# Maofei/loam_velodyne-1

Measured on AMD Instinct MI355X. Metric: scans/sec (odometry+mapping L-M solve) VLP-16 sweep, 1/2/4/8 MI355X, higher is better.
Workload: dtype fp32 (fp64 JtJ accumulation); 1 GPU; config4: independent VLP-16 problems (SR prev+cur, odometry L-M, mapping L-M); problems_per_gpu=1024, global_batch=1024, split=strong, parallelism=shard1

## Files before the change

### loam_velodyne-1_amd/csrc/dev_hooks.h

```cpp
#ifndef LOAM_DEV_HOOKS_H
#define LOAM_DEV_HOOKS_H

#include <stdint.h>

#ifdef __cplusplus
extern "C" {
#endif

typedef struct loam_dev_vg loam_dev_vg;

#define LOAM_DEV_VG_STACK 0
#define LOAM_DEV_VG_CUBES 1
#define LOAM_DEV_VG_SURROUND 2

typedef struct {
  const float* pts;
  int32_t total;
  int32_t nseg;
  const int32_t* begin;
  const int32_t* end;
  const float* leaf;
  const int32_t* nold;
  int32_t route;
  int32_t P;
// ... 15 lines not shown
#define LOAM_DEV_NN5_MAX_QUERIES 4096
#define LOAM_DEV_NN5_BATCH 0
#define LOAM_DEV_NN5_STREAM 1
#define LOAM_DEV_NN5_OVERFLOW 1
#define LOAM_DEV_NN5_PLAIN 2

typedef struct {
  const float* map;
  int32_t n_map;
  const float* queries;
  int32_t n_queries;
  const int32_t* seeds;
  const int32_t* distinct;
  int32_t form;
} loam_dev_nn5_job;

int loam_dev_nn5_create(int device, loam_dev_nn5** out);

int loam_dev_nn5_run(loam_dev_nn5* h, const loam_dev_nn5_job* job, int32_t* flat_idx, uint32_t* flat_dist,
                     int32_t* plain_idx, uint32_t* plain_dist, int32_t* flags, int32_t* counts);

int loam_dev_nn5_destroy(loam_dev_nn5* h);

#ifdef __cplusplus
}
#endif
#endif
```

### loam_velodyne-1_amd/csrc/engine.hpp

```cpp
#ifndef LOAM_ENGINE_HPP
#define LOAM_ENGINE_HPP

#include <hip/hip_runtime.h>
#include <stdint.h>

#include <cstring>
#include <string>

#include "../../include/loam/loam.h"
#include "imu.hpp"
#include "prof.hpp"

namespace loam {

enum : int {
  ERR_CAP_RING = 1,
  ERR_CAP_ROWS = 2,
  ERR_EMPTY = 4,
  ERR_CAP_MAP = 8,
  ERR_CAP_STACK = 16,
  ERR_VG_BITS = 32,
};

constexpr int kSrThreads = 512;
// ... 7 lines not shown
  int od_fused_max = 128;
  int mp_small_max = 4;
  int mp_fused_max = 1 << 20;
  int od_assoc_wg = 0;
  int fit_wg = 0;
  int graph = 0;
  int vg_merge = 1;
  int vg_merge_min = 12288;
  int vg_split = 1;
  int sr_ahead = 64;
  int step_pipe = 64;
  int pipe_mp_sets = 2;
  int od_graph = 1;
  int pipe_sr_sets = 3;
  int batch_streams = 1;
  int sr_ahead_at = -1;
  int od_sel_min = 64;
  int od_win_mono = 3;
  int od_win_mono_min = 2;
  int stream_defer = 1;
  int od_persist = 1;
  int mp_persist = 1;
  int od_moments_min = 64;
  bool get(const char* key, long long* v) {
    return set(key, 0, v);
  }
  bool set(const char* key, long long v, long long* read = nullptr) {
    struct K { const char* n; int* f; long long lo, hi; };
    const K ks[] = {{"od_small_max", &od_small_max, 0, 1 << 20}, {"stream_defer", &stream_defer, 0, 1}, {"pipe_sr_sets", &pipe_sr_sets, 2, 3}, {"od_graph", &od_graph, 0, 1},
                    {"od_fused_max", &od_fused_max, 0, 1 << 20},
                    {"mp_small_max", &mp_small_max, 0, 1 << 20}, {"mp_fused_max", &mp_fused_max, 0, 1 << 20},
                    {"od_assoc_wg", &od_assoc_wg, 0, 1024}, {"fit_wg", &fit_wg, 0, 256}, {"graph", &graph, 0, 1},
                    {"vg_merge", &vg_merge, 0, 1}, {"vg_merge_min", &vg_merge_min, 0, 1 << 20}, {"vg_split", &vg_split, 0, 3},
                    {"sr_ahead", &sr_ahead, 0, 1 << 20}, {"sr_ahead_at", &sr_ahead_at, -1, 2},
                    {"step_pipe", &step_pipe, 0, 1 << 20}, {"batch_streams", &batch_streams, 0, 1},
                    {"pipe_mp_sets", &pipe_mp_sets, 1, 2}, {"od_sel_min", &od_sel_min, 1, 1 << 20},
                    {"od_win_mono", &od_win_mono, 0, 3}, {"od_win_mono_min", &od_win_mono_min, 1, 1 << 20},
                    {"od_moments_min", &od_moments_min, 1, 1 << 30}, {"od_persist", &od_persist, 0, 1},
                    {"mp_persist", &mp_persist, 0, 1}};
    for (const K& k : ks)
      if (std::strcmp(key, k.n) == 0) {
        if (read) {
          *read = *k.f;
          return true;
        }
        if (v < k.lo || v > k.hi) return false;
        *k.f = (int)v;
        return true;
      }
    return false;
  }
};

struct SrBuffers {
  int S = 0, cap = 0, R = 0;
  float4* raw = nullptr;
  int* raw_n = nullptr;
  float* tmp_ori = nullptr;
  uint8_t* tmp_sid = nullptr;
  int* tilecnt = nullptr;
  int* tileF = nullptr;
  int* ring_sync = nullptr;
// ... 141 lines not shown
```

### loam_velodyne-1_amd/csrc/od.hip

```cpp
#include "dev_common.hpp"
#include "od.hpp"
#include "pose_math.hpp"

using namespace loamdev;


#ifndef LOAM_ASSOC_SKIP
#define LOAM_ASSOC_SKIP 0
#endif
#ifndef LOAM_ASSOC_PHASE
#define LOAM_ASSOC_PHASE 0
#endif
#if (LOAM_ASSOC_SKIP != 0 || LOAM_ASSOC_PHASE != 0) && !defined(LOAM_EXPERIMENT_BUILD)
#error "LOAM_ASSOC_SKIP / LOAM_ASSOC_PHASE are diagnostic (wrong results / partial counters): tools/build_variant.sh only"
#endif

namespace loam {
#ifdef LOAM_PHASES
__device__ PhaseAcc g_ph_od = {~0ull, 0ull, 0ull, {{0}}};
#endif


namespace {

// ... 286 lines not shown
  hipLaunchKernelGGL(k_hash_scan, dim3(1, P, 2), dim3(1024), 0, st, hp);
  hipLaunchKernelGGL(k_hash_scatter, dim3(kHashGrid, P, 2), dim3(256), 0, st, hp);
}

namespace {


LOAM_D float box_d2(const float4& lo, const float4& hi, const float4& s) {
  const float gx = fmaxf(fmaxf(lo.x - s.x, s.x - hi.x), 0.0f);
  const float gy = fmaxf(fmaxf(lo.y - s.y, s.y - hi.y), 0.0f);
  const float gz = fmaxf(fmaxf(lo.z - s.z, s.z - hi.z), 0.0f);
  return sqdist(gx, gy, gz, 0.0f, 0.0f, 0.0f);
}

LOAM_D bool window_member(int j, int r, int c, int scan, int fwd_end, bool corner, bool same) {
  if (j > c) return j < fwd_end && r <= scan + 2 && (corner ? r > scan : (same ? r <= scan : r > scan));
  return j < c && r >= scan - 2 && (corner ? r < scan : (same ? r >= scan : r < scan));
}

struct WinBound {
  float same = 25.0f, other = 25.0f;
};

LOAM_D uint64_t wave_hash_nn(const int* start, const float4* hp, int T, const float4* cloud, const float4* ch,
                             int n, float h, float inv_h, float4 q, float bound, int* cells, int& wpts, int& wbox,
                             int kind = -1, int fwd_end = 0, bool mono = false, WinBound* wb = nullptr) {
  const int lane = lane_id();
  const int cx = cell_of(q.x, inv_h), cy = cell_of(q.y, inv_h), cz = cell_of(q.z, inv_h);
  int bucket = -1, b0 = 0, cnt = 0;
  if (lane < 27 && T > 0) {
    const int dx = lane % 3 - 1, dy = (lane / 3) % 3 - 1, dz = lane / 9 - 1;
    const float4 lo = make_float4((float)(cx + dx) * h, (float)(cy + dy) * h, (float)(cz + dz) * h, 0.0f);
    const float4 hi = make_float4((float)(cx + dx + 1) * h, (float)(cy + dy + 1) * h, (float)(cz + dz + 1) * h, 0.0f);
    const float bd = box_d2(lo, hi, q);
    if (h != 1.0f || (bd < 1.0f && bd <= bound)) {
      bucket = (int)(cell_hash(cx + dx, cy + dy, cz + dz) & (uint32_t)(T - 1));
      const int2 rg = load_pair(start + bucket);
      b0 = rg.x;
      cnt = rg.y - b0;
      LOAM_CHECK(b0 >= 0 && cnt >= 0 && b0 + cnt <= n, b0, cnt);
    }
  }
  const int incl = wave_incl_scan_x(cnt);
  const int total = __builtin_amdgcn_readlane(incl, 63);
  if (LOAM_ASSOC_PHASE == 0 || LOAM_ASSOC_PHASE == 1) wpts += total;
  if (lane < 32) { cells[lane] = lane < 27 ? incl - cnt : 0x7fffffff; cells[32 + lane] = b0; }
// ... 21 lines not shown
  if (best != ~0ull && __uint_as_float((uint32_t)(best >> 32)) < h * h) {
    if (kind >= 0 && mono && D(__uint_as_float((uint32_t)(best >> 32))) < 25) {
      const int c = (int)((uint32_t)best >> 8), scan = (int)((uint32_t)best & 255u);
      float ms = 3.4e38f, mo = 3.4e38f;
      for (int t = lane; t < total; t += 64) {
        const float4 a = t == lane ? a0 : cand(t);
        const uint32_t tag = (uint32_t)__float_as_int(a.w);
        const int j = (int)(tag & 0xffffffu), r = (int)(tag >> 24);
        const float d = sqdist(a.x, a.y, a.z, q.x, q.y, q.z);
        if (kind == 0) {
          if (window_member(j, r, c, scan, fwd_end, true, false)) mo = fminf(mo, d);
        } else if (window_member(j, r, c, scan, fwd_end, false, true)) {
          ms = fminf(ms, d);
        } else if (window_member(j, r, c, scan, fwd_end, false, false)) {
          mo = fminf(mo, d);
        }
      }
      wb->same = fminf(wb->same, wave_min_f_x(ms));
      wb->other = fminf(wb->other, wave_min_f_x(mo));
    }
    return best;
  }
  if (LOAM_ASSOC_SKIP & 2) return best;
  best = ~0ull;
  const int nch = (n + kChunk - 1) / kChunk;
  for (int k0 = 0; k0 < nch; k0 += 64) {
    const int k = k0 + lane;
    float bd = 0.0f;
    if (k < nch) bd = box_d2(ch[2 * k], ch[2 * k + 1], q);
    const bool need = k < nch && bd < 25.0f && bd <= bound;
    uint64_t nb = __ballot(need);
    wbox += min(64, nch - k0);
    while (nb) {
      const int c = k0 + __ffsll((unsigned long long)nb) - 1;
      nb &= nb - 1;
      if (LOAM_ASSOC_PHASE == 0 || LOAM_ASSOC_PHASE == 2) wpts += min(kChunk, n - c * kChunk);
      const int t = c * kChunk + lane;
      if (lane < kChunk && t < n) {
        const float4 a = cloud[t];
        const float d = sqdist(a.x, a.y, a.z, q.x, q.y, q.z);
        const uint64_t key = ((uint64_t)fkey(d) << 32) | ((uint32_t)t << 8) | (uint32_t)(int)a.w;
        best = key < best ? key : best;
      }
    }
  }
  return wave_min_u64_x(best);
}

#ifndef LOAM_WIN_INFLIGHT
#define LOAM_WIN_INFLIGHT 1
#endif
constexpr int kWinInFlight = LOAM_WIN_INFLIGHT;
template <typename F>
LOAM_D void wave_window(const float4* L, const float4* ch, int c, int end, int dir, int scan, float4 sel, float bs,
                        float bo, int& wpts, int& wbox, F f) {
  const int lane = lane_id();
  auto stop_ring = [&](int r) { return dir > 0 ? r > scan + 2 : r < scan - 2; };
  auto scan_pts = [&](int j0, int cnt, float4 a) {
    if (LOAM_ASSOC_PHASE == 0 || LOAM_ASSOC_PHASE == 3) wpts += cnt;
    const int j = j0 + dir * lane;
    const bool inr = lane < cnt;
    const int r = (int)a.w;
    const uint64_t mb = __ballot(inr && stop_ring(r));
    const int limit = mb ? __ffsll((unsigned long long)mb) - 1 : 64;
    if (inr && lane < limit) {
      const float d = sqdist(a.x, a.y, a.z, sel.x, sel.y, sel.z);
      if (d < 25) f(j, r, d);
    }
    return mb != 0;
// ... 279 lines not shown
  ist[kIsNanSkips] = 0;
  ist[kIsGathered] = 0;
  ist[kIsBoxes] = 0;
  b.done[p] = 0;
  if (p == 0 && b.P == 1) ++b.ls_epoch[0];
}

__global__ __launch_bounds__(kOdThreads) void k_od_sel(OdBuffers b, FeatView f) {
  const XcdBlock blk = xcd_block();
  const int p = blk.y;
  const int* ist = b.istate + (size_t)p * kOdStateInts;
  if (!ist[kIsActive] || ist[kIsStop]) return;
  const float* st = b.state + (size_t)p * kOdStateFloats;
  float T[6];
#pragma unroll
  for (int k = 0; k < 6; ++k) T[k] = st[k];
  const int nc = f.count(p, 0), nq = nc + f.count(p, 2);
  const int q = blk.x * kOdThreads + threadIdx.x;
  if (q >= nq) return;
  const float4 po = q < nc ? f.sharp[(size_t)p * f.sharp_stride + q] : f.flat[(size_t)p * f.flat_stride + (q - nc)];
  b.sel[(size_t)p * b.cap_q + q] = loampose::transform_to_start(T, po);
}

template <bool SEL>
LOAM_D void od_assoc_wave(const OdBuffers& b, const FeatView& f, int p, int last_buf, int q0, int G, const float* T,
                          bool seeded, int* cells, float4* bq_s4, float4* bq_d, int4* bq_j, const int* rsC,
                          const int* rsS, int& wpts, int& wbox) {
  const int lane = lane_id();
  const int nc = f.count(p, 0), ns = f.count(p, 2), nq = nc + ns;
  const size_t lp = (size_t)last_buf * b.P + p;
  const int C = b.nlast[(p * kOdBufs + last_buf) * 2 + 0], S = b.nlast[(p * kOdBufs + last_buf) * 2 + 1];
  const float4* CL = b.lastC + lp * b.capC;
  const float4* SL = b.lastS + lp * b.capS;
  int* ind = b.ind + (size_t)p * 3 * b.cap_q;
  const bool use_mono = b.P >= b.tune.od_win_mono_min && (b.tune.od_win_mono & (seeded ? 2 : 1)) != 0;
  const bool tight = LOAM_WIN_TIGHTEN == 1 || (LOAM_WIN_TIGHTEN == 2 && !seeded);
  const int hCT = b.hC_T[last_buf * b.P + p], hST = b.hS_T[last_buf * b.P + p];
  const bool monoC = b.mono[lp * 2 + 0] != 0, monoS = b.mono[lp * 2 + 1] != 0;
  for (int i0 = 0; q0 + i0 * G < nq; i0 += 64) {
    {
      const int ql = q0 + (i0 + lane) * G;
      if (ql < nq) {
        float4 s4;
        if constexpr (SEL) {
          const float4 po = ql < nc ? f.sharp[(size_t)p * f.sharp_stride + ql] : f.flat[(size_t)p * f.flat_stride + (ql - nc)];
          s4 = loampose::transform_to_start(T, po);
        } else {
          s4 = b.sel[(size_t)p * b.cap_q + ql];
        }
        const float4* Lc = ql < nc ? CL : SL;
        int j[3] = {-1, -1, -1};
        if (seeded) {
#pragma unroll
          for (int k = 0; k < 3; ++k) j[k] = ind[k * b.cap_q + ql];
        }
        float4 sp[3];
#pragma unroll
        for (int k = 0; k < 3; ++k) sp[k] = j[k] >= 0 ? Lc[j[k]] : make_float4(0, 0, 0, 0);
        const float nnb = j[0] >= 0 ? sqdist(sp[0].x, sp[0].y, sp[0].z, s4.x, s4.y, s4.z) : 3.4e38f;
        const float d1 = sqdist(sp[1].x, sp[1].y, sp[1].z, s4.x, s4.y, s4.z);
        const float d2 = sqdist(sp[2].x, sp[2].y, sp[2].z, s4.x, s4.y, s4.z);
        bq_s4[lane] = s4;
        bq_j[lane] = make_int4(j[0], j[1], j[2], (int)sp[1].w | ((int)sp[2].w << 16));
        bq_d[lane] = make_float4(nnb, d1, d2, 0.0f);
      }
    }
    __builtin_amdgcn_wave_barrier();
    const int nb = min(64, (nq - q0 + G - 1) / G - i0);
    for (int i = 0; i < nb; ++i) {
      const int q = q0 + (i0 + i) * G;
      const float4 s4 = bq_s4[i];
      const int4 jj = bq_j[i];
      const float4 dd = bq_d[i];
      const int j1 = jj.y, j2 = jj.z, r1 = jj.w & 0xffff, r2 = jj.w >> 16;
      const float nnb = dd.x, d1 = dd.y, d2 = dd.z;
      int i1, i2, i3 = -1;
      WinBound wb;
      if (q < nc && monoC && use_mono) {
        const float4* ch = b.cC + lp * 2 * chunks_of(b.capC);
        const uint64_t nn = wave_hash_nn(b.hC_start + lp * (b.tC + 1), b.hC_pts + lp * b.capC, hCT, CL, ch, C, 1.0f,
                                         1.0f, s4, nnb, cells, wpts, wbox, seeded || !LOAM_WIN_WB ? -1 : 0, min(nc, C), true, &wb);
        i1 = i2 = -1;
        if (nn != ~0ull && D(__uint_as_float((uint32_t)(nn >> 32))) < 25) {
          const int c = (int)((uint32_t)nn >> 8), scan = (int)((uint32_t)nn & 255u), fe = min(nc, C);
          i1 = c;
          uint64_t k2 = ~0ull, k3 = mono_seed_key(rsC, c, scan, fe, j1, d1, false);
          wave_window_mono(CL, b.fC + lp * 2 * subs_of(b.capC), rsC, c, scan, fe, s4, false, wb, tight, k2, k3, wpts, wbox);
          if (k3 != ~0ull) i2 = mono_decode(c, k3);
        }
      } else if (q >= nc && monoS && use_mono) {
        const float4* ch = b.cS + lp * 2 * chunks_of(b.capS);
        const uint64_t nn = wave_hash_nn(b.hS_start + lp * (b.tS + 1), b.hS_pts + lp * b.capS, hST, SL, ch, S, 1.0f,
                                         1.0f, s4, nnb, cells, wpts, wbox, seeded || !LOAM_WIN_WB ? -1 : 1, min(ns, S), true, &wb);
        i1 = i2 = -1;
        if (nn != ~0ull && D(__uint_as_float((uint32_t)(nn >> 32))) < 25) {
          const int c = (int)((uint32_t)nn >> 8), scan = (int)((uint32_t)nn & 255u), fe = min(ns, S);
          i1 = c;
          uint64_t k2 = mono_seed_key(rsS, c, scan, fe, j1, d1, true);
          uint64_t k3 = mono_seed_key(rsS, c, scan, fe, j2, d2, false);
          wave_window_mono(SL, b.fS + lp * 2 * subs_of(b.capS), rsS, c, scan, fe, s4, true, wb, tight, k2, k3, wpts, wbox);
          if (k2 != ~0ull) i2 = mono_decode(c, k2);
          if (k3 != ~0ull) i3 = mono_decode(c, k3);
        }
      } else if (q < nc) {
        const float4* ch = b.cC + lp * 2 * chunks_of(b.capC);
        const uint64_t nn = wave_hash_nn(b.hC_start + lp * (b.tC + 1), b.hC_pts + lp * b.capC, hCT, CL, ch, C, 1.0f,
                                         1.0f, s4, nnb, cells, wpts, wbox, seeded ? -1 : 0, min(nc, C), monoC, &wb);
        wave_assoc_corner(CL, ch, min(nc, C), nn, s4, j1, r1, d1, wb, monoC, i1, i2, wpts, wbox);
      } else {
        const float4* ch = b.cS + lp * 2 * chunks_of(b.capS);
        const uint64_t nn = wave_hash_nn(b.hS_start + lp * (b.tS + 1), b.hS_pts + lp * b.capS, hST, SL, ch, S, 1.0f,
                                         1.0f, s4, nnb, cells, wpts, wbox, seeded ? -1 : 1, min(ns, S), monoS, &wb);
        wave_assoc_surf(SL, ch, min(ns, S), nn, s4, j1, r1, d1, j2, r2, d2, wb, monoS, i1, i2, i3, wpts, wbox);
      }
      if (lane == 0) {
        LOAM_CHECK(q < b.cap_q && p < b.P, q, p);
        LOAM_CHECK(i1 < (q < nc ? C : S) && i2 < (q < nc ? C : S) && i3 < S, i1, i2);
        ind[q] = i1;
        ind[b.cap_q + q] = i2;
        ind[2 * b.cap_q + q] = i3;
      }
    }
    __builtin_amdgcn_wave_barrier();
  }
}

template <bool COUNT, bool SEL>
__global__ __launch_bounds__(kAsThreads) __attribute__((amdgpu_waves_per_eu(SEL ? 1 : 8))) void k_od_assoc(OdBuffers b, FeatView f, int last_buf) {
  const XcdBlock blk = xcd_block();
  const int p = blk.y, lane = lane_id(), w = threadIdx.x >> 6;
  const int* ist = b.istate + (size_t)p * kOdStateInts;
  if (!ist[kIsActive] || ist[kIsStop]) return;
  __shared__ int cells[kAsWaves][64];
  __shared__ float4 bq_s4[kAsWaves][64], bq_d[kAsWaves][64];
  __shared__ int4 bq_j[kAsWaves][64];
  __shared__ int rsC[kRingTab], rsS[kRingTab];
  static_assert(kAsWaves == 1, "the ring tables are loaded by the workgroup's one wave");
  const size_t lp = (size_t)last_buf * b.P + p;
  for (int r = lane; r < kRingTab; r += 64) {
    rsC[r] = b.rstart[lp * 2 * kRingTab + r];
    rsS[r] = b.rstart[lp * 2 * kRingTab + kRingTab + r];
  }
  __builtin_amdgcn_wave_barrier();
  float T[6];
  if constexpr (SEL) {
    const float* st = b.state + (size_t)p * kOdStateFloats;
#pragma unroll
    for (int k = 0; k < 6; ++k) T[k] = st[k];
  }
  int wpts = 0, wbox = 0;
  const bool seeded = ist[kIsIters] > 0;
  od_assoc_wave<SEL>(b, f, p, last_buf, blk.x * kAsWaves + w, gridDim.x * kAsWaves, T, seeded, cells[w], bq_s4[w],
                     bq_d[w], bq_j[w], rsC, rsS, wpts, wbox);
  if (COUNT && lane == 0) {
    if (wpts) atomicAdd((int*)&ist[kIsGathered], wpts);
    if (wbox) atomicAdd((int*)&ist[kIsBoxes], wbox);
  }
}

LOAM_D void od_step(const OdBuffers& b, int p, int iter, const double* tot, float* AtA, float* AtB, float* X,
                    float* lm_ws, int* lm_iws, float* jE, float* jV) {
  const int lane = lane_id();
  int* ist = b.istate + (size_t)p * kOdStateInts;
  float* st = b.state + (size_t)p * kOdStateFloats;
  const int nrows = (int)tot[27];
  int c_rows = 0, degen = 0, c_deg = 0, c_nan = 0;
  float T[6] = {0, 0, 0, 0, 0, 0};
  if (lane == 0) {
    const int c_assoc = ist[kIsAssoc];
    c_rows = ist[kIsRows];
    degen = ist[kIsDegenerate];
    c_deg = ist[kIsDegSteps];
    c_nan = ist[kIsNanSkips];
#pragma unroll
    for (int q = 0; q < 6; ++q) T[q] = st[q];
    ist[kIsIters] = iter + 1;
// ... 817 lines not shown
  A(&b.istate_set[0], (size_t)P * kOdStateInts * sizeof(int));
  A(&b.istate_set[1], (size_t)P * kOdStateInts * sizeof(int));
  A(&b.istate_set[2], (size_t)P * kOdStateInts * sizeof(int));
  b.istate = b.istate_set[0];
  A(&b.lastC, (size_t)kOdBufs * P * b.capC * sizeof(float4));
  A(&b.lastS, (size_t)kOdBufs * P * b.capS * sizeof(float4));
  A(&b.fullEnd, (size_t)kOdBufs * P * b.capS * sizeof(float4));
  A(&b.nlast, (size_t)P * kOdBufs * 2 * sizeof(int));
  A(&b.nfullEnd, (size_t)P * kOdBufs * sizeof(int));
  A(&b.hC_start, (size_t)kOdBufs * P * (b.tC + 1) * sizeof(int));
  A(&b.hS_start, (size_t)kOdBufs * P * (b.tS + 1) * sizeof(int));
  A(&b.hC_fill, (size_t)P * b.tC * sizeof(int));
  A(&b.hS_fill, (size_t)P * b.tS * sizeof(int));
  A(&b.hC_pts, (size_t)kOdBufs * P * b.capC * sizeof(float4));
  A(&b.hS_pts, (size_t)kOdBufs * P * b.capS * sizeof(float4));
  A(&b.hC_T, (size_t)kOdBufs * P * sizeof(int));
  A(&b.cC, (size_t)kOdBufs * P * 2 * chunks_of(b.capC) * sizeof(float4));
  A(&b.cS, (size_t)kOdBufs * P * 2 * chunks_of(b.capS) * sizeof(float4));
  A(&b.fC, (size_t)kOdBufs * P * 2 * subs_of(b.capC) * sizeof(float4));
  A(&b.fS, (size_t)kOdBufs * P * 2 * subs_of(b.capS) * sizeof(float4));
  A(&b.hS_T, (size_t)kOdBufs * P * sizeof(int));
  A(&b.ind, (size_t)P * 3 * b.cap_q * sizeof(int));
  A(&b.sel, (size_t)P * b.cap_q * sizeof(float4));
  A(&b.q_cf, (size_t)P * max_iter * b.cap_q * sizeof(float4));
  A(&b.q_ok, (size_t)P * max_iter * b.cap_q * sizeof(int8_t));
  A(&b.mom, (size_t)P * kOdMom * b.cap_q * sizeof(double));
  A(&b.qa, (size_t)P * b.cap_q * 3 * sizeof(float4));
  A(&b.part, (size_t)P * b.gq * max_iter * 28 * sizeof(double));
  A(&b.done, (size_t)P * sizeof(int));
  A(&b.ls_part, (size_t)2 * kOdLsMaxG * 28 * sizeof(double));
  A(&b.ls_flag, (size_t)kOdLsMaxG * sizeof(unsigned long long));
  A(&b.ls_epoch, sizeof(unsigned long long));
  A(&b.mono, (size_t)kOdBufs * P * 2 * sizeof(int));
  A(&b.rstart, (size_t)kOdBufs * P * 2 * kRingTab * sizeof(int));
  if (A.err != hipSuccess) {
    od_free(b);
    return A.err;
  }
  if (A.err == hipSuccess) A.err = hipMemset(b.done, 0, (size_t)P * sizeof(int));
  if (A.err == hipSuccess) A.err = hipMemset(b.ls_flag, 0, (size_t)kOdLsMaxG * sizeof(unsigned long long));
  if (A.err == hipSuccess) A.err = hipMemset(b.ls_epoch, 0, sizeof(unsigned long long));
  for (int k = 0; k < 3; ++k)
    if (A.err == hipSuccess) A.err = hipMemset(b.state_set[k], 0, (size_t)P * kOdStateFloats * sizeof(float));
  for (int k = 0; k < 3; ++k)
    if (A.err == hipSuccess) A.err = hipMemset(b.istate_set[k], 0, (size_t)P * kOdStateInts * sizeof(int));
  if (A.err == hipSuccess) A.err = hipMemset(b.nlast, 0, (size_t)P * kOdBufs * 2 * sizeof(int));
  if (A.err == hipSuccess) A.err = hipMemset(b.nfullEnd, 0, (size_t)P * kOdBufs * sizeof(int));
  if (A.err == hipSuccess) A.err = hipMemset(b.hC_T, 0, (size_t)kOdBufs * P * sizeof(int));
  if (A.err == hipSuccess) A.err = hipMemset(b.hS_T, 0, (size_t)kOdBufs * P * sizeof(int));
  if (A.err != hipSuccess) od_free(b);
  return A.err;
}

void od_free(OdBuffers& b) {
  if (b.hash_pending && b.hash_done) (void)hipEventSynchronize(b.hash_done);
  if (b.hash_fork) (void)hipEventDestroy(b.hash_fork);
  if (b.hash_done) (void)hipEventDestroy(b.hash_done);
  void* ptrs[] = {b.state_set[0], b.state_set[1], b.state_set[2], b.istate_set[0], b.istate_set[1], b.istate_set[2], b.lastC, b.lastS, b.fullEnd, b.nlast, b.nfullEnd, b.hC_start,
                  b.hS_start, b.hC_fill, b.hS_fill, b.hC_pts, b.hS_pts, b.hC_T, b.hS_T, b.cC, b.cS,
                  b.ind, b.sel, b.q_cf, b.q_ok, b.mom, b.qa, b.part, b.done, b.mono, b.rstart, b.fC, b.fS,
                  b.ls_part, b.ls_flag, b.ls_epoch};
  for (void* q : ptrs)
    if (q) (void)hipFree(q);
  b = OdBuffers();
}

hipError_t od_build_hashes_deferred(OdBuffers& b, int buf, hipStream_t st, hipStream_t side) {
  hipError_t e = hipSuccess;
  if (!b.hash_fork) e = hipEventCreateWithFlags(&b.hash_fork, hipEventDisableTiming);
  if (e == hipSuccess && !b.hash_done) e = hipEventCreateWithFlags(&b.hash_done, hipEventDisableTiming);
  if (e == hipSuccess) e = hipEventRecord(b.hash_fork, st);
  if (e == hipSuccess) e = hipStreamWaitEvent(side, b.hash_fork, 0);
  if (e != hipSuccess) return e;
  od_build_hashes(b, buf, side);
  e = hipEventRecord(b.hash_done, side);
  if (e == hipSuccess) b.hash_pending = true;
  return e;
}

hipError_t od_wait_hashes(OdBuffers& b, hipStream_t st) {
  if (!b.hash_pending) return hipSuccess;
  b.hash_pending = false;
  return hipStreamWaitEvent(st, b.hash_done, 0);
// ... 34 lines not shown
  js.chunks = b.cS + (size_t)buf * b.P * 2 * chunks_of(b.capS);
  js.fine = b.fS + (size_t)buf * b.P * 2 * subs_of(b.capS);
  hash_build_pair(jc, js, b.P, st, true);
}

}

namespace loam {
void od_solve(const OdBuffers& b, const FeatView& f, int last_buf, hipStream_t st, Prof* prof, bool device_fini) {
  const int P = b.P;
  auto mark = [&](const char* n) { if (prof) prof->mark(n); };
  hipLaunchKernelGGL(k_od_begin, dim3((P + 255) / 256), dim3(256), 0, st, b, f);
  const Tuning& tn = b.tune;
  const int gls = P == 1 && tn.od_persist ? od_lm_stream_grid(b.cap_q) : 0;
  if (gls > 0) {
    hipLaunchKernelGGL(k_od_lm_stream, dim3(gls), dim3(kOdLsThreads), 0, st, b, f, last_buf);
    mark("k_od_lm_stream");
  }
  for (int it = 0; it < (gls > 0 ? 0 : b.max_iter); ++it) {
    if (it % 5 == 0) {
      const int ga = P >= 64 ? (tn.od_assoc_wg > 0 ? tn.od_assoc_wg : std::max(16, std::min(1024, b.cap_q / 9)))
                             : (b.cap_q + kAsWaves - 1) / kAsWaves;
      if (P >= tn.od_sel_min) {
        hipLaunchKernelGGL(k_od_sel, dim3(b.gq, P), dim3(kOdThreads), 0, st, b, f);
        if (prof) {
          hipLaunchKernelGGL((k_od_assoc<true, false>), dim3(ga, P), dim3(kAsThreads), 0, st, b, f, last_buf);
        } else {
          hipLaunchKernelGGL((k_od_assoc<false, false>), dim3(ga, P), dim3(kAsThreads), 0, st, b, f, last_buf);
        }
      } else {
        if (prof) hipLaunchKernelGGL((k_od_assoc<true, true>), dim3(ga, P), dim3(kAsThreads), 0, st, b, f, last_buf);
        else hipLaunchKernelGGL((k_od_assoc<false, true>), dim3(ga, P), dim3(kAsThreads), 0, st, b, f, last_buf);
      }
      mark("k_od_assoc");
    }
    if (P <= tn.od_small_max) {
      hipLaunchKernelGGL(k_od_rows_small, dim3(b.gq, P, it + 1), dim3(kOdThreads), 0, st, b, f, last_buf, it);
      mark("k_od_rows");
    } else {
      const bool mom = P >= tn.od_moments_min;
      if (P <= tn.od_fused_max) {
        if (mom) hipLaunchKernelGGL((k_od_rows_mom<true>), dim3(b.gq, P), dim3(kOdThreads), 0, st, b, f, last_buf, it);
        else hipLaunchKernelGGL((k_od_rows<true, 2>), dim3(b.gq, P), dim3(kOdThreads), 0, st, b, f, last_buf, it);
        mark("k_od_rows");
      } else {
        if (mom) hipLaunchKernelGGL((k_od_rows_mom<false>), dim3(b.gq, P), dim3(kOdThreads), 0, st, b, f, last_buf, it);
        else hipLaunchKernelGGL((k_od_rows<false, 2>), dim3(b.gq, P), dim3(kOdThreads), 0, st, b, f, last_buf, it);
        mark("k_od_rows");
        hipLaunchKernelGGL(k_od_step, dim3(P), dim3(64), 0, st, b, it, b.gq);
        mark("k_od_step");
      }
    }
  }
  if (device_fini) hipLaunchKernelGGL(k_od_fini, dim3((P + 63) / 64), dim3(64), 0, st, b, f);
}

void od_fini(const OdBuffers& b, const FeatView& f, hipStream_t st) {
  hipLaunchKernelGGL(k_od_fini, dim3((b.P + 63) / 64), dim3(64), 0, st, b, f);
}
}


#ifdef LOAM_PHASES
extern "C" int loam_debug_phases_od(unsigned long long* out) {
  if (hipDeviceSynchronize() != hipSuccess) return -1;
  return hipMemcpyFromSymbol(out, HIP_SYMBOL(loam::g_ph_od), sizeof(PhaseAcc)) == hipSuccess ? 0 : -1;
}
#endif
```

### loam_velodyne-1_amd/csrc/od.hpp

```cpp
#ifndef LOAM_OD_HPP
#define LOAM_OD_HPP

#include <hip/hip_runtime.h>
#include <stdint.h>

#include "engine.hpp"

namespace loam {

constexpr int kOdLsMaxG = 128;
#ifndef LOAM_OD_CHUNK
#define LOAM_OD_CHUNK 64
#endif
#ifndef LOAM_OD_END_WG
#define LOAM_OD_END_WG 16
#endif
constexpr int kOdEndWg = LOAM_OD_END_WG;
constexpr int kChunk = LOAM_OD_CHUNK;
__host__ __device__ inline int chunks_of(int cap) { return (cap + kChunk - 1) / kChunk; }
#ifndef LOAM_WIN_SUB
#define LOAM_WIN_SUB 32
#endif
constexpr int kSub = LOAM_WIN_SUB;
static_assert(kSub == 16 || kSub == 32 || kSub == 64, "sub-chunks of 16, 32 or 64 points");
// ... 56 lines not shown
  int* istate_set[3] = {nullptr, nullptr, nullptr};
  hipEvent_t hash_fork = nullptr, hash_done = nullptr;
  bool hash_pending = false;
  float* bk_state = nullptr;
  int* bk_istate = nullptr;
  float4* lastC = nullptr;
  float4* lastS = nullptr;
  float4* fullEnd = nullptr;
  int* nlast = nullptr;
  int* nfullEnd = nullptr;
  int* hC_start = nullptr;
  int* hS_start = nullptr;
  int* hC_fill = nullptr;
  int* hS_fill = nullptr;
  float4* hC_pts = nullptr;
  float4* hS_pts = nullptr;
  int* hC_T = nullptr;
  int* hS_T = nullptr;
  float4* cC = nullptr;
  float4* cS = nullptr;
  float4* fC = nullptr;
  float4* fS = nullptr;
  float4* sel = nullptr;
  int* ind = nullptr;
  float4* q_cf = nullptr;
  int8_t* q_ok = nullptr;
  float4* qa = nullptr;
  double* mom = nullptr;
  double* part = nullptr;
  int* done = nullptr;
  double* ls_part = nullptr;
  unsigned long long* ls_flag = nullptr;
  unsigned long long* ls_epoch = nullptr;
  int* mono = nullptr;
  int* rstart = nullptr;
  Tuning tune;
};

void hash_build_pair(const HashJob& a, const HashJob& b, int P, hipStream_t st, bool wide, bool spread = false);

__global__ void k_od_end(OdBuffers b, FeatView f, int dst, int mode, int do_full);

hipError_t od_alloc(OdBuffers& b, int P, int R, int cap_pts, int max_iter);
void od_free(OdBuffers& b);
void od_build_hashes(const OdBuffers& b, int buf, hipStream_t st);
hipError_t od_build_hashes_deferred(OdBuffers& b, int buf, hipStream_t st, hipStream_t side);
// ... 9 lines not shown
```

Measured before the change: 84970 scans/s.

## Precompute odometry nearest neighbours per lane before wave-level association

Adds a lane-per-query kernel that transforms each feature point and searches the 27 neighbouring hash cells in parallel, keeping several point loads in flight, then stores the nearest-neighbour key per query. The wave-per-query association kernel reuses that key and falls back to the chunked wave search only when the lane search found nothing within range. The aim is to take the serial wave-wide nearest-neighbour search off the association critical path, at the cost of an extra kernel launch, a per-query key buffer and a large shared-memory list per block. It also adds a device test hook that compares lane, wave and chunk results.

```diff
diff --git a/loam_velodyne-1_amd/csrc/dev_hooks.h b/loam_velodyne-1_amd/csrc/dev_hooks.h
--- a/loam_velodyne-1_amd/csrc/dev_hooks.h
+++ b/loam_velodyne-1_amd/csrc/dev_hooks.h
@@ -61,6 +61,26 @@
 
 int loam_dev_nn5_destroy(loam_dev_nn5* h);
 
+typedef struct loam_dev_od_nn loam_dev_od_nn;
+
+#define LOAM_DEV_OD_NN_MAX_CLOUD 16384
+#define LOAM_DEV_OD_NN_MAX_QUERIES 4096
+
+typedef struct {
+  const float* cloud;
+  int32_t n_cloud;
+  const float* queries;
+  int32_t n_queries;
+  const int32_t* seeds;
+} loam_dev_od_nn_job;
+
+int loam_dev_od_nn_create(int device, loam_dev_od_nn** out);
+
+int loam_dev_od_nn_run(loam_dev_od_nn* h, const loam_dev_od_nn_job* job, uint64_t* lane_key, uint64_t* wave_key,
+                       uint64_t* chunk_key, int32_t* left);
+
+int loam_dev_od_nn_destroy(loam_dev_od_nn* h);
+
 #ifdef __cplusplus
 }
 #endif
diff --git a/loam_velodyne-1_amd/csrc/engine.hpp b/loam_velodyne-1_amd/csrc/engine.hpp
--- a/loam_velodyne-1_amd/csrc/engine.hpp
+++ b/loam_velodyne-1_amd/csrc/engine.hpp
@@ -53,6 +53,8 @@
   int od_persist = 1;
   int mp_persist = 1;
   int od_moments_min = 64;
+  int od_nn_lane = 2;
+  int od_nn_lane_min = 512;
   bool get(const char* key, long long* v) {
     return set(key, 0, v);
   }
@@ -68,7 +70,8 @@
                     {"pipe_mp_sets", &pipe_mp_sets, 1, 2}, {"od_sel_min", &od_sel_min, 1, 1 << 20},
                     {"od_win_mono", &od_win_mono, 0, 3}, {"od_win_mono_min", &od_win_mono_min, 1, 1 << 20},
                     {"od_moments_min", &od_moments_min, 1, 1 << 30}, {"od_persist", &od_persist, 0, 1},
-                    {"mp_persist", &mp_persist, 0, 1}};
+                    {"mp_persist", &mp_persist, 0, 1}, {"od_nn_lane", &od_nn_lane, 0, 2},
+                    {"od_nn_lane_min", &od_nn_lane_min, 1, 1 << 20}};
     for (const K& k : ks)
       if (std::strcmp(key, k.n) == 0) {
         if (read) {
diff --git a/loam_velodyne-1_amd/csrc/od.hip b/loam_velodyne-1_amd/csrc/od.hip
--- a/loam_velodyne-1_amd/csrc/od.hip
+++ b/loam_velodyne-1_amd/csrc/od.hip
@@ -1,4 +1,7 @@
+#include <vector>
+
 #include "dev_common.hpp"
+#include "dev_hooks.h"
 #include "od.hpp"
 #include "pose_math.hpp"
 
@@ -332,6 +335,34 @@
   float same = 25.0f, other = 25.0f;
 };
 
+LOAM_D uint64_t wave_chunk_nn(const float4* cloud, const float4* ch, int n, float4 q, float bound, int& wpts,
+                              int& wbox) {
+  const int lane = lane_id();
+  uint64_t best = ~0ull;
+  const int nch = (n + kChunk - 1) / kChunk;
+  for (int k0 = 0; k0 < nch; k0 += 64) {
+    const int k = k0 + lane;
+    float bd = 0.0f;
+    if (k < nch) bd = box_d2(ch[2 * k], ch[2 * k + 1], q);
+    const bool need = k < nch && bd < 25.0f && bd <= bound;
+    uint64_t nb = __ballot(need);
+    wbox += min(64, nch - k0);
+    while (nb) {
+      const int c = k0 + __ffsll((unsigned long long)nb) - 1;
+      nb &= nb - 1;
+      if (LOAM_ASSOC_PHASE == 0 || LOAM_ASSOC_PHASE == 2) wpts += min(kChunk, n - c * kChunk);
+      const int t = c * kChunk + lane;
+      if (lane < kChunk && t < n) {
+        const float4 a = cloud[t];
+        const float d = sqdist(a.x, a.y, a.z, q.x, q.y, q.z);
+        const uint64_t key = ((uint64_t)fkey(d) << 32) | ((uint32_t)t << 8) | (uint32_t)(int)a.w;
+        best = key < best ? key : best;
+      }
+    }
+  }
+  return wave_min_u64_x(best);
+}
+
 LOAM_D uint64_t wave_hash_nn(const int* start, const float4* hp, int T, const float4* cloud, const float4* ch,
                              int n, float h, float inv_h, float4 q, float bound, int* cells, int& wpts, int& wbox,
                              int kind = -1, int fwd_end = 0, bool mono = false, WinBound* wb = nullptr) {
@@ -399,29 +430,108 @@
     return best;
   }
   if (LOAM_ASSOC_SKIP & 2) return best;
-  best = ~0ull;
-  const int nch = (n + kChunk - 1) / kChunk;
-  for (int k0 = 0; k0 < nch; k0 += 64) {
-    const int k = k0 + lane;
-    float bd = 0.0f;
-    if (k < nch) bd = box_d2(ch[2 * k], ch[2 * k + 1], q);
-    const bool need = k < nch && bd < 25.0f && bd <= bound;
-    uint64_t nb = __ballot(need);
-    wbox += min(64, nch - k0);
-    while (nb) {
-      const int c = k0 + __ffsll((unsigned long long)nb) - 1;
-      nb &= nb - 1;
-      if (LOAM_ASSOC_PHASE == 0 || LOAM_ASSOC_PHASE == 2) wpts += min(kChunk, n - c * kChunk);
-      const int t = c * kChunk + lane;
-      if (lane < kChunk && t < n) {
-        const float4 a = cloud[t];
-        const float d = sqdist(a.x, a.y, a.z, q.x, q.y, q.z);
-        const uint64_t key = ((uint64_t)fkey(d) << 32) | ((uint32_t)t << 8) | (uint32_t)(int)a.w;
+  return wave_chunk_nn(cloud, ch, n, q, bound, wpts, wbox);
+}
+
+constexpr uint64_t kNnLaneNone = ~0ull;
+#ifndef LOAM_LANE_NN_INFLIGHT
+#define LOAM_LANE_NN_INFLIGHT 4
+#endif
+constexpr int kLaneNnInFlight = LOAM_LANE_NN_INFLIGHT;
+constexpr int kLaneNnList = 27, kLaneNnGroup = 27;
+LOAM_D uint64_t nn_key(const float4& a, const float4& q) {
+  const float d = sqdist(a.x, a.y, a.z, q.x, q.y, q.z);
+  const uint32_t tag = (uint32_t)__float_as_int(a.w);
+  return ((uint64_t)fkey(d) << 32) | ((tag & 0xffffffu) << 8) | (tag >> 24);
+}
+template <int S>
+LOAM_D uint64_t lane_hash_nn(const int* start, const float4* hp, int T, int n, float4 q, float bound, uint32_t* lst,
+                             int& work) {
+  if (T <= 0) return kNnLaneNone;
+  const int cx = cell_of(q.x, 1.0f), cy = cell_of(q.y, 1.0f), cz = cell_of(q.z, 1.0f);
+  auto bucket_of = [&](int c, bool& need) {
+    const int dx = c % 3 - 1, dy = (c / 3) % 3 - 1, dz = c / 9 - 1;
+    const float4 lo = make_float4((float)(cx + dx), (float)(cy + dy), (float)(cz + dz), 0.0f);
+    const float4 hi = make_float4((float)(cx + dx + 1), (float)(cy + dy + 1), (float)(cz + dz + 1), 0.0f);
+    const float bd = box_d2(lo, hi, q);
+    need = bd < 1.0f && bd <= bound;
+    return (int)(cell_hash(cx + dx, cy + dy, cz + dz) & (uint32_t)(T - 1));
+  };
+  int nl = 0, total = 0;
+  bool fits = true;
+#pragma unroll
+  for (int g0 = 0; g0 < 27; g0 += kLaneNnGroup) {
+    int2 rg[kLaneNnGroup];
+#pragma unroll
+    for (int u = 0; u < kLaneNnGroup; ++u) {
+      if (g0 + u >= 27) break;
+      bool need;
+      const int bk = bucket_of(g0 + u, need);
+      rg[u] = make_int2(0, 0);
+      if (need) rg[u] = load_pair(start + bk);
+    }
+#pragma unroll
+    for (int u = 0; u < kLaneNnGroup; ++u) {
+      if (g0 + u >= 27) break;
+      const int cnt = rg[u].y - rg[u].x;
+      LOAM_CHECK(rg[u].x >= 0 && cnt >= 0 && rg[u].x + cnt <= n, rg[u].x, cnt);
+      if (cnt > 0) {
+        const uint32_t e = hash_rec(rg[u].x, cnt);
+        if (e == kRecNone || nl == kLaneNnList) {
+          fits = false;
+        } else {
+          lst[nl * S] = e;
+          ++nl;
+        }
+        total += cnt;
+      }
+    }
+  }
+  if (LOAM_ASSOC_PHASE == 0 || LOAM_ASSOC_PHASE == 1) work += total;
+  uint64_t best = kNnLaneNone;
+  if (fits) {
+    int ci = 1, left = 0, pos = 0;
+    uint32_t nx = lst[0];
+    auto next = [&]() {
+      if (left == 0) {
+        pos = (int)(nx & ((1u << 19) - 1));
+        left = (int)(nx >> 19);
+        nx = lst[min(ci, kLaneNnList - 1) * S];
+        ++ci;
+      }
+      --left;
+      return pos++;
+    };
+    for (int k = 0; k < total; k += kLaneNnInFlight) {
+      int idx[kLaneNnInFlight];
+#pragma unroll
+      for (int u = 0; u < kLaneNnInFlight; ++u) idx[u] = k + u < total ? next() : idx[0];
+      float4 a[kLaneNnInFlight];
+#pragma unroll
+      for (int u = 0; u < kLaneNnInFlight; ++u) {
+        LOAM_CHECK(idx[u] >= 0 && idx[u] < n, idx[u], n);
+        a[u] = hp[idx[u]];
+      }
+#pragma unroll
+      for (int u = 0; u < kLaneNnInFlight; ++u) {
+        const uint64_t key = nn_key(a[u], q);
         best = key < best ? key : best;
       }
     }
-  }
-  return wave_min_u64_x(best);
+  } else {
+#pragma unroll 1
+    for (int c = 0; c < 27; ++c) {
+      bool need;
+      const int bk = bucket_of(c, need);
+      if (!need) continue;
+      const int2 r = load_pair(start + bk);
+      for (int k = r.x; k < r.y; ++k) {
+        const uint64_t key = nn_key(hp[k], q);
+        best = key < best ? key : best;
+      }
+    }
+  }
+  return best != kNnLaneNone && __uint_as_float((uint32_t)(best >> 32)) < 1.0f ? best : kNnLaneNone;
 }
 
 #ifndef LOAM_WIN_INFLIGHT
@@ -747,10 +857,53 @@
   b.sel[(size_t)p * b.cap_q + q] = loampose::transform_to_start(T, po);
 }
 
+template <bool COUNT>
+__global__ __launch_bounds__(kOdThreads) void k_od_sel_nn(OdBuffers b, FeatView f, int last_buf) {
+  __shared__ uint32_t lst[kLaneNnList * kOdThreads];
+  const XcdBlock blk = xcd_block();
+  const int p = blk.y;
+  int* ist = b.istate + (size_t)p * kOdStateInts;
+  if (!ist[kIsActive] || ist[kIsStop]) return;
+  const float* st = b.state + (size_t)p * kOdStateFloats;
+  float T[6];
+#pragma unroll
+  for (int k = 0; k < 6; ++k) T[k] = st[k];
+  const int nc = f.count(p, 0), nq = nc + f.count(p, 2);
+  const int q = blk.x * kOdThreads + threadIdx.x;
+  int work = 0;
+  if (q < nq) {
+    const bool corner = q < nc;
+    const float4 po = corner ? f.sharp[(size_t)p * f.sharp_stride + q] : f.flat[(size_t)p * f.flat_stride + (q - nc)];
+    const float4 s4 = loampose::transform_to_start(T, po);
+    b.sel[(size_t)p * b.cap_q + q] = s4;
+    const size_t lp = (size_t)last_buf * b.P + p;
+    const float4* L = corner ? b.lastC + lp * b.capC : b.lastS + lp * b.capS;
+    const int n = b.nlast[(p * kOdBufs + last_buf) * 2 + (corner ? 0 : 1)];
+    float bound = 3.4e38f;
+    if (ist[kIsIters] > 0) {
+      const int j0 = b.ind[(size_t)p * 3 * b.cap_q + q];
+      if (j0 >= 0) {
+        const float4 sp = L[j0];
+        bound = sqdist(sp.x, sp.y, sp.z, s4.x, s4.y, s4.z);
+      }
+    }
+    const int* start = corner ? b.hC_start + lp * (b.tC + 1) : b.hS_start + lp * (b.tS + 1);
+    const float4* hp = corner ? b.hC_pts + lp * b.capC : b.hS_pts + lp * b.capS;
+    const int hT = corner ? b.hC_T[last_buf * b.P + p] : b.hS_T[last_buf * b.P + p];
+    b.nnw[(size_t)p * b.cap_q + q] = lane_hash_nn<kOdThreads>(start, hp, hT, n, s4, bound, lst + threadIdx.x, work);
+  }
+  if constexpr (COUNT) {
+#pragma unroll
+    for (int o = 32; o > 0; o >>= 1) work += __shfl_xor(work, o, 64);
+    if (lane_id() == 0 && work) atomicAdd(&ist[kIsGathered], work);
+  }
+}
+
 template <bool SEL>
 LOAM_D void od_assoc_wave(const OdBuffers& b, const FeatView& f, int p, int last_buf, int q0, int G, const float* T,
                           bool seeded, int* cells, float4* bq_s4, float4* bq_d, int4* bq_j, const int* rsC,
-                          const int* rsS, int& wpts, int& wbox) {
+                          const int* rsS, int& wpts, int& wbox, const uint64_t* nnw = nullptr,
+                          uint64_t* bq_nn = nullptr) {
   const int lane = lane_id();
   const int nc = f.count(p, 0), ns = f.count(p, 2), nq = nc + ns;
   const size_t lp = (size_t)last_buf * b.P + p;
@@ -788,6 +941,7 @@
         bq_s4[lane] = s4;
         bq_j[lane] = make_int4(j[0], j[1], j[2], (int)sp[1].w | ((int)sp[2].w << 16));
         bq_d[lane] = make_float4(nnb, d1, d2, 0.0f);
+        if (nnw) bq_nn[lane] = nnw[ql];
       }
     }
     __builtin_amdgcn_wave_barrier();
@@ -801,10 +955,22 @@
       const float nnb = dd.x, d1 = dd.y, d2 = dd.z;
       int i1, i2, i3 = -1;
       WinBound wb;
+      auto wave_nn = [&](bool corner, int kind, int fe, bool mono) {
+        const float4* L = corner ? CL : SL;
+        const float4* ch = corner ? b.cC + lp * 2 * chunks_of(b.capC) : b.cS + lp * 2 * chunks_of(b.capS);
+        const int n = corner ? C : S;
+        if (nnw && kind < 0) {
+          const uint64_t w = bq_nn[i];
+          if (w != kNnLaneNone || (LOAM_ASSOC_SKIP & 2)) return w;
+          return wave_chunk_nn(L, ch, n, s4, nnb, wpts, wbox);
+        }
+        return corner ? wave_hash_nn(b.hC_start + lp * (b.tC + 1), b.hC_pts + lp * b.capC, hCT, L, ch, n, 1.0f, 1.0f, s4,
+                                     nnb, cells, wpts, wbox, kind, fe, mono, &wb)
+                      : wave_hash_nn(b.hS_start + lp * (b.tS + 1), b.hS_pts + lp * b.capS, hST, L, ch, n, 1.0f, 1.0f, s4,
+                                     nnb, cells, wpts, wbox, kind, fe, mono, &wb);
+      };
       if (q < nc && monoC && use_mono) {
-        const float4* ch = b.cC + lp * 2 * chunks_of(b.capC);
-        const uint64_t nn = wave_hash_nn(b.hC_start + lp * (b.tC + 1), b.hC_pts + lp * b.capC, hCT, CL, ch, C, 1.0f,
-                                         1.0f, s4, nnb, cells, wpts, wbox, seeded || !LOAM_WIN_WB ? -1 : 0, min(nc, C), true, &wb);
+        const uint64_t nn = wave_nn(true, seeded || !LOAM_WIN_WB ? -1 : 0, min(nc, C), true);
         i1 = i2 = -1;
         if (nn != ~0ull && D(__uint_as_float((uint32_t)(nn >> 32))) < 25) {
           const int c = (int)((uint32_t)nn >> 8), scan = (int)((uint32_t)nn & 255u), fe = min(nc, C);
@@ -814,9 +980,7 @@
           if (k3 != ~0ull) i2 = mono_decode(c, k3);
         }
       } else if (q >= nc && monoS && use_mono) {
-        const float4* ch = b.cS + lp * 2 * chunks_of(b.capS);
-        const uint64_t nn = wave_hash_nn(b.hS_start + lp * (b.tS + 1), b.hS_pts + lp * b.capS, hST, SL, ch, S, 1.0f,
-                                         1.0f, s4, nnb, cells, wpts, wbox, seeded || !LOAM_WIN_WB ? -1 : 1, min(ns, S), true, &wb);
+        const uint64_t nn = wave_nn(false, seeded || !LOAM_WIN_WB ? -1 : 1, min(ns, S), true);
         i1 = i2 = -1;
         if (nn != ~0ull && D(__uint_as_float((uint32_t)(nn >> 32))) < 25) {
           const int c = (int)((uint32_t)nn >> 8), scan = (int)((uint32_t)nn & 255u), fe = min(ns, S);
@@ -829,13 +993,11 @@
         }
       } else if (q < nc) {
         const float4* ch = b.cC + lp * 2 * chunks_of(b.capC);
-        const uint64_t nn = wave_hash_nn(b.hC_start + lp * (b.tC + 1), b.hC_pts + lp * b.capC, hCT, CL, ch, C, 1.0f,
-                                         1.0f, s4, nnb, cells, wpts, wbox, seeded ? -1 : 0, min(nc, C), monoC, &wb);
+        const uint64_t nn = wave_nn(true, seeded ? -1 : 0, min(nc, C), monoC);
         wave_assoc_corner(CL, ch, min(nc, C), nn, s4, j1, r1, d1, wb, monoC, i1, i2, wpts, wbox);
       } else {
         const float4* ch = b.cS + lp * 2 * chunks_of(b.capS);
-        const uint64_t nn = wave_hash_nn(b.hS_start + lp * (b.tS + 1), b.hS_pts + lp * b.capS, hST, SL, ch, S, 1.0f,
-                                         1.0f, s4, nnb, cells, wpts, wbox, seeded ? -1 : 1, min(ns, S), monoS, &wb);
+        const uint64_t nn = wave_nn(false, seeded ? -1 : 1, min(ns, S), monoS);
         wave_assoc_surf(SL, ch, min(ns, S), nn, s4, j1, r1, d1, j2, r2, d2, wb, monoS, i1, i2, i3, wpts, wbox);
       }
       if (lane == 0) {
@@ -851,12 +1013,13 @@
 }
 
 template <bool COUNT, bool SEL>
-__global__ __launch_bounds__(kAsThreads) __attribute__((amdgpu_waves_per_eu(SEL ? 1 : 8))) void k_od_assoc(OdBuffers b, FeatView f, int last_buf) {
+__global__ __launch_bounds__(kAsThreads) __attribute__((amdgpu_waves_per_eu(SEL ? 1 : 8))) void k_od_assoc(OdBuffers b, FeatView f, int last_buf, int nn_lane) {
   const XcdBlock blk = xcd_block();
   const int p = blk.y, lane = lane_id(), w = threadIdx.x >> 6;
   const int* ist = b.istate + (size_t)p * kOdStateInts;
   if (!ist[kIsActive] || ist[kIsStop]) return;
   __shared__ int cells[kAsWaves][64];
+  __shared__ uint64_t bq_nn[kAsWaves][64];
   __shared__ float4 bq_s4[kAsWaves][64], bq_d[kAsWaves][64];
   __shared__ int4 bq_j[kAsWaves][64];
   __shared__ int rsC[kRingTab], rsS[kRingTab];
@@ -876,7 +1039,8 @@
   int wpts = 0, wbox = 0;
   const bool seeded = ist[kIsIters] > 0;
   od_assoc_wave<SEL>(b, f, p, last_buf, blk.x * kAsWaves + w, gridDim.x * kAsWaves, T, seeded, cells[w], bq_s4[w],
-                     bq_d[w], bq_j[w], rsC, rsS, wpts, wbox);
+                     bq_d[w], bq_j[w], rsC, rsS, wpts, wbox,
+                     !SEL && nn_lane ? b.nnw + (size_t)p * b.cap_q : nullptr, bq_nn[w]);
   if (COUNT && lane == 0) {
     if (wpts) atomicAdd((int*)&ist[kIsGathered], wpts);
     if (wbox) atomicAdd((int*)&ist[kIsBoxes], wbox);
@@ -1740,6 +1904,7 @@
   A(&b.hS_T, (size_t)kOdBufs * P * sizeof(int));
   A(&b.ind, (size_t)P * 3 * b.cap_q * sizeof(int));
   A(&b.sel, (size_t)P * b.cap_q * sizeof(float4));
+  A(&b.nnw, (size_t)P * b.cap_q * sizeof(uint64_t));
   A(&b.q_cf, (size_t)P * max_iter * b.cap_q * sizeof(float4));
   A(&b.q_ok, (size_t)P * max_iter * b.cap_q * sizeof(int8_t));
   A(&b.mom, (size_t)P * kOdMom * b.cap_q * sizeof(double));
@@ -1776,7 +1941,7 @@
   if (b.hash_done) (void)hipEventDestroy(b.hash_done);
   void* ptrs[] = {b.state_set[0], b.state_set[1], b.state_set[2], b.istate_set[0], b.istate_set[1], b.istate_set[2], b.lastC, b.lastS, b.fullEnd, b.nlast, b.nfullEnd, b.hC_start,
                   b.hS_start, b.hC_fill, b.hS_fill, b.hC_pts, b.hS_pts, b.hC_T, b.hS_T, b.cC, b.cS,
-                  b.ind, b.sel, b.q_cf, b.q_ok, b.mom, b.qa, b.part, b.done, b.mono, b.rstart, b.fC, b.fS,
+                  b.ind, b.sel, b.nnw, b.q_cf, b.q_ok, b.mom, b.qa, b.part, b.done, b.mono, b.rstart, b.fC, b.fS,
                   b.ls_part, b.ls_flag, b.ls_epoch};
   for (void* q : ptrs)
     if (q) (void)hipFree(q);
@@ -1857,15 +2022,18 @@
       const int ga = P >= 64 ? (tn.od_assoc_wg > 0 ? tn.od_assoc_wg : std::max(16, std::min(1024, b.cap_q / 9)))
                              : (b.cap_q + kAsWaves - 1) / kAsWaves;
       if (P >= tn.od_sel_min) {
-        hipLaunchKernelGGL(k_od_sel, dim3(b.gq, P), dim3(kOdThreads), 0, st, b, f);
+        const int nnl = P >= tn.od_nn_lane_min && (tn.od_nn_lane == 2 || (tn.od_nn_lane == 1 && it > 0)) ? 1 : 0;
+        if (!nnl) hipLaunchKernelGGL(k_od_sel, dim3(b.gq, P), dim3(kOdThreads), 0, st, b, f);
+        else if (prof) hipLaunchKernelGGL(k_od_sel_nn<true>, dim3(b.gq, P), dim3(kOdThreads), 0, st, b, f, last_buf);
+        else hipLaunchKernelGGL(k_od_sel_nn<false>, dim3(b.gq, P), dim3(kOdThreads), 0, st, b, f, last_buf);
         if (prof) {
-          hipLaunchKernelGGL((k_od_assoc<true, false>), dim3(ga, P), dim3(kAsThreads), 0, st, b, f, last_buf);
+          hipLaunchKernelGGL((k_od_assoc<true, false>), dim3(ga, P), dim3(kAsThreads), 0, st, b, f, last_buf, nnl);
         } else {
-          hipLaunchKernelGGL((k_od_assoc<false, false>), dim3(ga, P), dim3(kAsThreads), 0, st, b, f, last_buf);
+          hipLaunchKernelGGL((k_od_assoc<false, false>), dim3(ga, P), dim3(kAsThreads), 0, st, b, f, last_buf, nnl);
         }
       } else {
-        if (prof) hipLaunchKernelGGL((k_od_assoc<true, true>), dim3(ga, P), dim3(kAsThreads), 0, st, b, f, last_buf);
-        else hipLaunchKernelGGL((k_od_assoc<false, true>), dim3(ga, P), dim3(kAsThreads), 0, st, b, f, last_buf);
+        if (prof) hipLaunchKernelGGL((k_od_assoc<true, true>), dim3(ga, P), dim3(kAsThreads), 0, st, b, f, last_buf, 0);
+        else hipLaunchKernelGGL((k_od_assoc<false, true>), dim3(ga, P), dim3(kAsThreads), 0, st, b, f, last_buf, 0);
       }
       mark("k_od_assoc");
     }
@@ -1896,6 +2064,171 @@
 }
 
 
+namespace loam {
+namespace {
+struct DevOdNn {
+  const float4 *cloud, *hp, *ch, *qs;
+  const int *start, *seeds;
+  int n, T, nq;
+  uint64_t *lane, *wave, *chunk;
+};
+LOAM_D float dev_od_nn_bound(const DevOdNn& d, int q, float4 s4) {
+  const int j0 = d.seeds ? d.seeds[q] : -1;
+  if (j0 < 0) return 3.4e38f;
+  const float4 sp = d.cloud[j0];
+  return sqdist(sp.x, sp.y, sp.z, s4.x, s4.y, s4.z);
+}
+__global__ __launch_bounds__(kOdThreads) void k_dev_od_nn_lane(DevOdNn d) {
+  __shared__ uint32_t lst[kLaneNnList * kOdThreads];
+  const int q = blockIdx.x * kOdThreads + threadIdx.x;
+  if (q >= d.nq) return;
+  const float4 s4 = d.qs[q];
+  int work = 0;
+  d.lane[q] = lane_hash_nn<kOdThreads>(d.start, d.hp, d.T, d.n, s4, dev_od_nn_bound(d, q, s4), lst + threadIdx.x, work);
+}
+__global__ __launch_bounds__(64) void k_dev_od_nn_wave(DevOdNn d) {
+  __shared__ int cells[64];
+  const int q = blockIdx.x;
+  const float4 s4 = d.qs[q];
+  const float bound = dev_od_nn_bound(d, q, s4);
+  int wpts = 0, wbox = 0;
+  const uint64_t w = wave_hash_nn(d.start, d.hp, d.T, d.cloud, d.ch, d.n, 1.0f, 1.0f, s4, bound, cells, wpts, wbox);
+  const uint64_t c = wave_chunk_nn(d.cloud, d.ch, d.n, s4, bound, wpts, wbox);
+  if (lane_id() == 0) {
+    d.wave[q] = w;
+    d.chunk[q] = c;
+  }
+}
+}
+}
+
+struct loam_dev_od_nn {
+  int device = 0;
+  hipStream_t st = nullptr;
+  float4 *cloud = nullptr, *hpts = nullptr, *hpts2 = nullptr, *qs = nullptr, *chunks = nullptr, *chunks2 = nullptr;
+  int *start = nullptr, *start2 = nullptr, *fill = nullptr, *fill2 = nullptr, *count = nullptr, *tsize = nullptr;
+  int* seeds = nullptr;
+  uint64_t* keys = nullptr;
+};
+
+namespace {
+void dev_od_nn_free(loam_dev_od_nn* h) {
+  void* ptrs[] = {h->cloud, h->hpts, h->hpts2, h->qs, h->chunks, h->chunks2, h->start, h->start2,
+                  h->fill, h->fill2, h->count, h->tsize, h->seeds, h->keys};
+  for (void* q : ptrs)
+    if (q) (void)hipFree(q);
+  if (h->st) (void)hipStreamDestroy(h->st);
+  delete h;
+}
+}
+
+extern "C" int loam_dev_od_nn_create(int device, loam_dev_od_nn** out) {
+  if (!out) return LOAM_E_INVAL;
+  *out = nullptr;
+  int ndev = 0;
+  if (hipGetDeviceCount(&ndev) != hipSuccess || ndev == 0) return LOAM_E_HIP;
+  if (device < 0 || device >= ndev) return LOAM_E_INVAL;
+  if (hipSetDevice(device) != hipSuccess) return LOAM_E_HIP;
+  loam_dev_od_nn* h = new loam_dev_od_nn();
+  h->device = device;
+  const size_t M = LOAM_DEV_OD_NN_MAX_CLOUD, Q = LOAM_DEV_OD_NN_MAX_QUERIES;
+  loam::DevAlloc A;
+  A(&h->cloud, M * sizeof(float4));
+  A(&h->hpts, M * sizeof(float4));
+  A(&h->hpts2, M * sizeof(float4));
+  A(&h->qs, Q * sizeof(float4));
+  A(&h->chunks, 2 * (size_t)loam::chunks_of((int)M) * sizeof(float4));
+  A(&h->chunks2, 2 * (size_t)loam::chunks_of((int)M) * sizeof(float4));
+  A(&h->start, (M + 1) * sizeof(int));
+  A(&h->start2, (M + 1) * sizeof(int));
+  A(&h->fill, M * sizeof(int));
+  A(&h->fill2, M * sizeof(int));
+  A(&h->count, 2 * sizeof(int));
+  A(&h->tsize, 2 * sizeof(int));
+  A(&h->seeds, Q * sizeof(int));
+  A(&h->keys, 3 * Q * sizeof(uint64_t));
+  hipError_t e = A.err;
+  if (e == hipSuccess) e = hipStreamCreate(&h->st);
+  if (e != hipSuccess) {
+    dev_od_nn_free(h);
+    return e == hipErrorOutOfMemory ? LOAM_E_NOMEM : LOAM_E_HIP;
+  }
+  *out = h;
+  return LOAM_OK;
+}
+
+extern "C" int loam_dev_od_nn_run(loam_dev_od_nn* h, const loam_dev_od_nn_job* job, uint64_t* lane_key,
+                                  uint64_t* wave_key, uint64_t* chunk_key, int32_t* left) {
+  using namespace loam;
+  if (!h || !job || !lane_key || !wave_key || !left) return LOAM_E_INVAL;
+  const int n = job->n_cloud, nq = job->n_queries;
+  if (!job->cloud || !job->queries || n < 1 || n > LOAM_DEV_OD_NN_MAX_CLOUD || nq < 1 || nq > LOAM_DEV_OD_NN_MAX_QUERIES)
+    return LOAM_E_INVAL;
+  if (job->seeds)
+    for (int k = 0; k < nq; ++k)
+      if (job->seeds[k] < -1 || job->seeds[k] >= n) return LOAM_E_INVAL;
+  for (int k = 0; k < n; ++k) {
+    const float r = job->cloud[4 * k + 3];
+    if (!(r >= 0.0f && r < 256.0f)) return LOAM_E_INVAL;
+  }
+  hipStream_t st = h->st;
+  auto up = [&](void* d, const void* s, size_t bytes) { return hipMemcpyAsync(d, s, bytes, hipMemcpyHostToDevice, st); };
+  const int cnt2[2] = {n, 0};
+  hipError_t e = hipSetDevice(h->device);
+  if (e == hipSuccess) e = up(h->cloud, job->cloud, (size_t)n * sizeof(float4));
+  if (e == hipSuccess) e = up(h->qs, job->queries, (size_t)nq * sizeof(float4));
+  if (e == hipSuccess) e = up(h->count, cnt2, sizeof(cnt2));
+  if (e == hipSuccess && job->seeds) e = up(h->seeds, job->seeds, (size_t)nq * sizeof(int));
+  if (e != hipSuccess) {
+    (void)hipStreamSynchronize(st);
+    return LOAM_E_HIP;
+  }
+  HashJob hc;
+  hc.pts = h->cloud; hc.pts_stride = LOAM_DEV_OD_NN_MAX_CLOUD; hc.pts_off = nullptr; hc.pts_off_stride = 0;
+  hc.count = h->count; hc.count_stride_bytes = 2 * sizeof(int);
+  hc.start = h->start; hc.fill = h->fill; hc.out = h->hpts; hc.tsize = h->tsize; hc.tmax = LOAM_DEV_OD_NN_MAX_CLOUD;
+  hc.inv_h = 1.0f;
+  hc.shift = 1;
+  hc.chunks = h->chunks;
+  HashJob hs = hc;
+  hs.count = h->count + 1; hs.start = h->start2; hs.fill = h->fill2; hs.out = h->hpts2; hs.tsize = h->tsize + 1;
+  hs.chunks = h->chunks2;
+  hash_build_pair(hc, hs, 1, st, true);
+  int T = 0;
+  e = hipMemcpyAsync(&T, h->tsize, sizeof(int), hipMemcpyDeviceToHost, st);
+  if (e == hipSuccess) e = hipStreamSynchronize(st);
+  if (e != hipSuccess) return LOAM_E_HIP;
+  DevOdNn d;
+  d.cloud = h->cloud; d.hp = h->hpts; d.ch = h->chunks; d.qs = h->qs;
+  d.start = h->start; d.seeds = job->seeds ? h->seeds : nullptr;
+  d.n = n; d.T = T; d.nq = nq;
+  const size_t Q = LOAM_DEV_OD_NN_MAX_QUERIES;
+  d.lane = h->keys; d.wave = h->keys + Q; d.chunk = h->keys + 2 * Q;
+  hipLaunchKernelGGL(k_dev_od_nn_lane, dim3((nq + kOdThreads - 1) / kOdThreads), dim3(kOdThreads), 0, st, d);
+  hipLaunchKernelGGL(k_dev_od_nn_wave, dim3(nq), dim3(64), 0, st, d);
+  e = hipGetLastError();
+  std::vector<uint64_t> ck((size_t)nq);
+  if (e == hipSuccess) e = hipMemcpyAsync(lane_key, d.lane, (size_t)nq * sizeof(uint64_t), hipMemcpyDeviceToHost, st);
+  if (e == hipSuccess) e = hipMemcpyAsync(wave_key, d.wave, (size_t)nq * sizeof(uint64_t), hipMemcpyDeviceToHost, st);
+  if (e == hipSuccess) e = hipMemcpyAsync(ck.data(), d.chunk, (size_t)nq * sizeof(uint64_t), hipMemcpyDeviceToHost, st);
+  const hipError_t es = hipStreamSynchronize(st);
+  if (e == hipSuccess) e = es;
+  if (e != hipSuccess) return LOAM_E_HIP;
+  for (int q = 0; q < nq; ++q) {
+    left[q] = lane_key[q] == ~0ull ? 1 : 0;
+    if (chunk_key) chunk_key[q] = ck[q];
+  }
+  return LOAM_OK;
+}
+
+extern "C" int loam_dev_od_nn_destroy(loam_dev_od_nn* h) {
+  if (!h) return LOAM_E_INVAL;
+  (void)hipSetDevice(h->device);
+  if (h->st) (void)hipStreamSynchronize(h->st);
+  dev_od_nn_free(h);
+  return LOAM_OK;
+}
+
 #ifdef LOAM_PHASES
 extern "C" int loam_debug_phases_od(unsigned long long* out) {
   if (hipDeviceSynchronize() != hipSuccess) return -1;
diff --git a/loam_velodyne-1_amd/csrc/od.hpp b/loam_velodyne-1_amd/csrc/od.hpp
--- a/loam_velodyne-1_amd/csrc/od.hpp
+++ b/loam_velodyne-1_amd/csrc/od.hpp
@@ -102,6 +102,7 @@
   float4* fC = nullptr;
   float4* fS = nullptr;
   float4* sel = nullptr;
+  uint64_t* nnw = nullptr;
   int* ind = nullptr;
   float4* q_cf = nullptr;
   int8_t* q_ok = nullptr;
```

After: 86480 scans/s, median of 6. 1.8% higher.
